# archinetai/audio-diffusion-pytorch

Measured on NVIDIA B200. Metric: audio-seconds/sec (2ch, 2^18 len) VSampler 50-step, higher is better.
Workload: dtype bf16

## Files before the change

audio_diffusion_pytorch_b200/csrc/conv_gemm.cu:

```cuda
#include <type_traits>

#include "common.cuh"
#include "ptx.cuh"

namespace adp {

int g_debug[8] = {2, 1, 0, 0, 0, 0, 0, 0};

constexpr int kBM = 128;
constexpr int kMaxStages = 8;
constexpr int kMaxGroups = 8;

struct Gemm2Params {
  __nv_bfloat16* out;
  const __nv_bfloat16* residual;
  const float* bias;
  const float* gate;
  double* stats;
  int B, T, tiles_per_batch, c_in, ldo;
  int n_pad, n_valid;
  int ntaps, tap_off0, up_factor;
  int groups, group_size, group_shift;
  int out_fp32, ld_gate;
  int n_tiles_n, total_tiles, tiles_per_cta;
// ... 558 lines not shown
  if (BN != 128 || SW != 128 || XF || g_debug[0] != 3) return false;
  const int taps = a.up_factor > 1 ? 2 : a.ntaps;
  const long m_tiles = (long)a.B * ((a.T + kBM - 1) / kBM);
  return m_tiles >= 2 && (a.c_in / 64) * taps >= 8;
}

template <int BN, int SW, bool XF>
static int launch_gemm2(const adp_conv_gemm_args& a, cudaStream_t stream) {
  if constexpr (BN == 128 && SW == 128 && !XF) {
    if (use_pairs<BN, SW, XF>(a)) {
      const long m_pairs = ((long)a.B * ((a.T + kBM - 1) / kBM) + 1) / 2;
      const long total = m_pairs * (a.phases * a.n_pad / BN);
      if (g_debug[7] == 0 && 2 * total <= 2L * num_sms()) return launch_gemm2_ew<BN, SW, XF, 8, 2>(a, stream, 1);
      return launch_gemm2_ew<BN, SW, XF, 4, 2>(a, stream, 1);
    }
  }
  return launch_gemm2_ew<BN, SW, XF, 4>(a, stream, 0);
}

template <int BN, int SW, bool XF, int EW, int CG>
static int launch_gemm2_ew(const adp_conv_gemm_args& a, cudaStream_t stream, int occ_in) {
  constexpr int BK = SW / 2;
  constexpr int WN = BN / CG;
  const int tiles_per_batch = (a.T + kBM - 1) / kBM;
  const bool up = a.up_factor > 1;
  const int max_taps = up ? 2 : a.ntaps;
  const int span = up ? 1 : a.ntaps - 1;
  const int a_rows = kBM + span;
  const int k_chunks = a.c_in / BK;

  Gemm2Params p;
  p.a_sub_bytes = (a_rows * SW + 1023) / 1024 * 1024;
  p.w_sub_bytes = (WN * SW + 1023) / 1024 * 1024;
  p.max_taps = max_taps;
  const int chunk_bytes = p.a_sub_bytes + max_taps * p.w_sub_bytes;

  const int w_iters = k_chunks * max_taps;
  int occ = 1;
  if (BN <= 64 && w_iters <= 8) occ = 3;
  else if (BN <= 128 && w_iters <= 12) occ = 2;
  if (XF && occ > (BN <= 64 ? 2 : 1)) occ = BN <= 64 ? 2 : 1;
  if (g_debug[3] > 0) occ = g_debug[3];
  if (occ_in > 0) occ = occ_in;
  const int tmem_occ = 512 / (2 * (BN < 32 ? 32 : BN));
  if (occ > tmem_occ) occ = tmem_occ;
  auto budget_of = [](int o) {
    return (o == 1 ? (EW == 8 ? 204 : 196) : (o == 2 ? (XF ? 92 : 96) : 60)) * 1024;
  };
  while (occ > 1 && budget_of(occ) < 2 * chunk_bytes) --occ;
  if constexpr (EW == 4 && !XF && BN >= 64 && CG == 1) {
    const long total = (long)a.B * tiles_per_batch * (a.phases * a.n_pad / BN);
    if (g_debug[7] == 0 && ((occ == 1 && total <= 2L * num_sms()) || total <= (long)num_sms()))
      return launch_gemm2_ew<BN, SW, XF, 8>(a, stream, 1);
  }
  const int budget = budget_of(occ);
  int kc = 1;
  while (kc * 2 <= 4 && k_chunks % (kc * 2) == 0 && kc * max_taps * (BK / 16) < 8 &&
         2 * (kc * 2) * chunk_bytes <= budget)
    kc *= 2;
  if (g_debug[5] > 0 && k_chunks % g_debug[5] == 0) kc = g_debug[5];
  p.kc = kc;
  p.k_stages = k_chunks / kc;
  p.stage_bytes = kc * chunk_bytes;
  int n_stages = budget / p.stage_bytes;
  if (n_stages > kMaxStages) n_stages = kMaxStages;
  if (n_stages < 2)
    return set_error("adp_conv_gemm: stage of %d bytes does not fit (BN=%d)", p.stage_bytes, BN);
  p.n_stages = n_stages;
  const size_t smem = static_cast<size_t>(n_stages) * p.stage_bytes + 1024;

  CUtensorMap tmA, tmW;
  {
    const uint64_t dims[3] = {(uint64_t)a.c_in, (uint64_t)a.T, (uint64_t)a.B};
    const uint64_t strides[2] = {(uint64_t)a.lda * 2, (uint64_t)a.T * a.lda * 2};
    const uint32_t box[3] = {(uint32_t)BK, (uint32_t)a_rows, 1};
    if (int e = make_tmap_bf16(&tmA, a.a, 3, dims, strides, box, SW)) return e;
  }
  {
    const uint64_t dims[2] = {(uint64_t)a.k_total, (uint64_t)a.phases * a.n_pad};
    const uint64_t strides[1] = {(uint64_t)a.k_total * 2};
    const uint32_t box[2] = {(uint32_t)BK, (uint32_t)WN};
    if (int e = make_tmap_bf16(&tmW, a.w, 2, dims, strides, box, SW)) return e;
  }

  static SmemAttrCache smem_cache;
  ADP_CUDA(ensure_dyn_smem(conv_gemm2_kernel<BN, SW, XF, EW, CG>, smem, smem_cache));

  p.out = static_cast<__nv_bfloat16*>(a.out);
  p.residual = static_cast<const __nv_bfloat16*>(a.residual);
  p.bias = a.bias;
  p.gate = a.gate;
  p.stats = a.stats;
  p.B = a.B;
  p.T = a.T;
  p.tiles_per_batch = tiles_per_batch;
  p.c_in = a.c_in;
  p.ldo = a.ldo;
  p.n_pad = a.n_pad;
  p.n_valid = a.n_valid;
  p.ntaps = a.ntaps;
  p.tap_off0 = a.tap_off[0];
  p.up_factor = a.up_factor;
  p.groups = a.stats ? a.groups : 0;
  p.group_size = a.stats ? a.n_valid / a.groups : 1;
  p.group_shift = -1;
  for (int sft = 0; sft < 16; ++sft)
    if ((1 << sft) == p.group_size) p.group_shift = sft;
  p.out_fp32 = a.out_fp32;
  p.ld_gate = a.ld_gate > 0 ? a.ld_gate : a.n_valid;
  p.n_tiles_n = a.phases * a.n_pad / BN;
  p.total_tiles = (a.B * tiles_per_batch + CG - 1) / CG * p.n_tiles_n;
  p.a_rows = a_rows;
  p.dbg = g_debug[4];
  p.early_w = g_debug[2];
  p.gn_stats = a.gn_stats;
  p.gn_gamma = a.gn_gamma;
  p.gn_beta = a.gn_beta;
  p.gn_eps = a.gn_eps;
  p.gn_groups = a.gn_groups > 0 ? a.gn_groups : 1;

  const int slots = occ * num_sms() / CG;
  int grid = p.total_tiles < slots ? p.total_tiles : slots;
  p.tiles_per_cta = (p.total_tiles + grid - 1) / grid;
  grid = (p.total_tiles + p.tiles_per_cta - 1) / p.tiles_per_cta;
  ADP_CUDA(launch_k_cluster(conv_gemm2_kernel<BN, SW, XF, EW, CG>, dim3(grid * CG),
                            dim3(64 + 32 * EW + (XF ? 256 : 0)), smem, stream, CG, tmA, tmW, p));
  ADP_LAUNCH_CHECK();
  return 0;
}

template <int SW>
static int dispatch_bn2(const adp_conv_gemm_args& a, int bn, cudaStream_t s) {
  if (a.gn_stats) {
    switch (bn) {
      case 16: return launch_gemm2<16, SW, true>(a, s);
      case 32: return launch_gemm2<32, SW, true>(a, s);
      case 64: return launch_gemm2<64, SW, true>(a, s);
      case 128: return launch_gemm2<128, SW, true>(a, s);
      case 256: return launch_gemm2<256, SW, true>(a, s);
    }
  }
  switch (bn) {
    case 16: return launch_gemm2<16, SW, false>(a, s);
    case 32: return launch_gemm2<32, SW, false>(a, s);
    case 64: return launch_gemm2<64, SW, false>(a, s);
    case 128: return launch_gemm2<128, SW, false>(a, s);
    case 256: return launch_gemm2<256, SW, false>(a, s);
  }
  return set_error("adp_conv_gemm: unsupported N tile %d", bn);
}

}

namespace adp { extern int g_mid_threads; }

extern "C" int adp_debug_set(int key, int value) {
  if (key == 8) {
    if (value != 128 && value != 256) return adp::set_error("adp_debug_set: key 8 takes 128 or 256");
    adp::g_mid_threads = value;
    return 0;
  }
  if (key < 0 || key >= 8) return adp::set_error("adp_debug_set: bad key %d", key);
  adp::g_debug[key] = value;
  if (key == 6) adp::g_pdl = value;
  return 0;
}

extern "C" int adp_conv_gemm(const adp_conv_gemm_args* args, adp_stream_t stream) {
  using namespace adp;
  ADP_CHECK(args != nullptr, "adp_conv_gemm: null args");
  const adp_conv_gemm_args& a = *args;
  ADP_CHECK(a.a && a.w && a.out, "adp_conv_gemm: null a/w/out");
  ADP_CHECK(a.B > 0 && a.T > 0, "adp_conv_gemm: bad B=%d T=%d", a.B, a.T);
  ADP_CHECK(a.c_in >= 16 && a.c_in % 16 == 0, "adp_conv_gemm: c_in=%d must be a multiple of 16",
            a.c_in);
  ADP_CHECK(a.lda % 8 == 0 && a.ldo % 8 == 0 && a.k_total % 8 == 0 && a.lda >= a.c_in,
            "adp_conv_gemm: pitches lda=%d ldo=%d k_total=%d must be multiples of 8", a.lda, a.ldo,
            a.k_total);
  ADP_CHECK(a.n_valid > 0 && a.n_valid % 8 == 0 && a.n_valid <= a.n_pad && a.n_pad % 16 == 0,
            "adp_conv_gemm: n_valid=%d n_pad=%d", a.n_valid, a.n_pad);
  ADP_CHECK(a.phases >= 1, "adp_conv_gemm: phases=%d", a.phases);
  ADP_CHECK(a.ld_gate % 4 == 0, "adp_conv_gemm: ld_gate=%d must be a multiple of 4", a.ld_gate);
  if (a.up_factor > 1) {
    ADP_CHECK(a.phases == a.up_factor, "adp_conv_gemm: phases (%d) != up_factor (%d)", a.phases,
              a.up_factor);
    ADP_CHECK(a.k_total >= 2 * a.c_in, "adp_conv_gemm: upsample weights need 2 tap slots");
  } else {
    ADP_CHECK(a.ntaps >= 1 && a.ntaps <= 3 && a.phases == 1, "adp_conv_gemm: ntaps=%d phases=%d",
              a.ntaps, a.phases);
    ADP_CHECK(a.k_total >= a.ntaps * a.c_in, "adp_conv_gemm: k_total too small");
    for (int i = 1; i < a.ntaps; ++i)
      ADP_CHECK(a.tap_off[i] == a.tap_off[i - 1] + 1,
                "adp_conv_gemm: tap offsets must be consecutive and ascending");
  }
  if (a.out_fp32) {
    ADP_CHECK(!a.residual && !a.stats, "adp_conv_gemm: out_fp32 excludes residual/stats");
  }
  if (a.gn_stats) {
    ADP_CHECK(a.c_in <= 1024, "adp_conv_gemm: fused GroupNorm supports c_in <= 1024");
    ADP_CHECK(a.gn_gamma && a.gn_beta && a.gn_groups > 0 && a.c_in % a.gn_groups == 0 && a.lda == a.c_in,
              "adp_conv_gemm: fused GroupNorm needs gamma/beta, groups | c_in and a dense input");
  }
  if (a.stats) {
    ADP_CHECK(a.groups > 0 && a.groups <= kMaxGroups && a.n_valid % a.groups == 0,
              "adp_conv_gemm: groups=%d n_valid=%d (fused statistics handle <= %d groups)",
              a.groups, a.n_valid, kMaxGroups);
  }
  int bn = a.block_n;
  if (bn == 0) {
    const long m_tiles = (long)a.B * ((a.T + kBM - 1) / kBM);
    bn = 16;
    for (int cand = 128; cand >= 16; cand >>= 1) {
      if (a.n_pad % cand) continue;
      const long tiles = m_tiles * (a.phases * a.n_pad / cand);
      if (tiles >= 96 || cand <= 64) { bn = cand; break; }
    }
  }
  ADP_CHECK(a.n_pad % bn == 0, "adp_conv_gemm: N tile %d does not divide n_pad %d", bn, a.n_pad);
  cudaStream_t s = as_stream(stream);
  if (a.c_in % 64 == 0) return dispatch_bn2<128>(a, bn, s);
  if (a.c_in % 32 == 0) return dispatch_bn2<64>(a, bn, s);
  return dispatch_bn2<32>(a, bn, s);
}
```

audio_diffusion_pytorch_b200/csrc/mid_conv.cu:

```cuda
#include "common.cuh"
#include "ptx.cuh"

namespace adp {

__device__ __forceinline__ void ldsm_x4(uint32_t addr, uint32_t (&r)[4]) {
  asm volatile("ldmatrix.sync.aligned.m8n8.x4.shared.b16 {%0,%1,%2,%3}, [%4];"
               : "=r"(r[0]), "=r"(r[1]), "=r"(r[2]), "=r"(r[3]) : "r"(addr));
}
__device__ __forceinline__ void mma_bf16_16816(float (&d)[4], const uint32_t (&a)[4], uint32_t b0,
                                               uint32_t b1) {
  asm volatile(
      "mma.sync.aligned.m16n8k16.row.col.f32.bf16.bf16.f32 {%0,%1,%2,%3}, {%4,%5,%6,%7}, {%8,%9}, "
      "{%0,%1,%2,%3};"
      : "+f"(d[0]), "+f"(d[1]), "+f"(d[2]), "+f"(d[3])
      : "r"(a[0]), "r"(a[1]), "r"(a[2]), "r"(a[3]), "r"(b0), "r"(b1));
}

template <int C, int NTH>
struct MidCfg {
  static constexpr int TB = (C == 32 ? 256 : 128) * NTH / 256;
  static constexpr int TPR = NTH / TB;
  static constexpr int RPW = TB / (NTH / 32);
  static constexpr int RS = C * 2 + 16;
  static constexpr int WS = 3 * C * 2 + 16;
  static constexpr int MB = RPW / 16;
  static constexpr int NT = C / 8;
  static constexpr int OS = C + 4;
  static constexpr int LPR = C / 8;
  static constexpr int ER = TB * LPR / NTH;
  static constexpr int X_BYTES = (TB + 2) * RS;
  static constexpr int O_BYTES = TB * OS * 4;
  static constexpr int W_BYTES = C * WS;
  static constexpr int SMEM = X_BYTES + O_BYTES + W_BYTES;
};

template <int C, int NTH>
__global__ void __launch_bounds__(NTH, 512 / NTH) mid_conv_kernel(const adp_narrow_conv_args a) {
  using Cfg = MidCfg<C, NTH>;
  constexpr int TB = Cfg::TB, TPR = Cfg::TPR, RS = Cfg::RS, WS = Cfg::WS, MB = Cfg::MB, NT = Cfg::NT;
  constexpr int OS = Cfg::OS, LPR = Cfg::LPR, ER = Cfg::ER, RPW = Cfg::RPW;
  pdl_launch_dependents();
  pdl_wait();
  extern __shared__ __align__(128) uint8_t smem[];
  uint8_t* s_x = smem;
  float* s_o = reinterpret_cast<float*>(smem + Cfg::X_BYTES);
  uint8_t* s_w = smem + Cfg::X_BYTES + Cfg::O_BYTES;
  __shared__ __align__(16) float s_ga[C], s_de[C];
  __shared__ __align__(16) float s_sc[C], s_sh[C];
  __shared__ float s_bias[C];
  __shared__ float s_stats[2 * 64];
  const int b = blockIdx.y;
  const int tid = threadIdx.x;
  const int warp = tid >> 5, lane = tid & 31;
  const int g = lane >> 2, q = lane & 3;
  const bool has_res = a.residual != nullptr, has_film = a.scale_shift != nullptr;

  if (tid < 128) s_stats[tid] = 0.f;
  if (a.w_packed) {
    constexpr int VPRW = 3 * C * 2 / 16;
    const uint4* wp = static_cast<const uint4*>(a.w_packed);
    for (int i = tid; i < C * VPRW; i += NTH) {
      const int co = i / VPRW, v = i - co * VPRW;
      *reinterpret_cast<uint4*>(s_w + co * WS + v * 16) = __ldg(wp + i);
    }
  } else {
    for (int pidx = tid; pidx < C * C; pidx += NTH) {
      const int co = pidx / C, ci = pidx % C;
      const float* src = a.w + static_cast<size_t>(pidx) * 3;
#pragma unroll
      for (int tap = 0; tap < 3; ++tap)
        *reinterpret_cast<__nv_bfloat16*>(s_w + co * WS + (tap * C + ci) * 2) = __float2bfloat16(src[tap]);
    }
  }
  if (tid < C) {
    const int c = tid;
    const int gsz = C / a.groups, gi = c / gsz;
    const double inv_n = 1.0 / (static_cast<double>(gsz) * a.T);
    const double sm = a.stats_in[(static_cast<size_t>(b) * a.groups + gi) * 2];
    const double sq = a.stats_in[(static_cast<size_t>(b) * a.groups + gi) * 2 + 1];
    const double mean = sm * inv_n;
    const float var = fmaxf(static_cast<float>(sq * inv_n - mean * mean), 0.f);
    const float ga = a.gamma[c] * rsqrtf(var + a.gn_eps);
    s_ga[c] = ga;
    s_de[c] = a.beta[c] - static_cast<float>(mean) * ga;
    s_bias[c] = a.bias ? a.bias[c] : 0.f;
    const float* ss = has_film ? a.scale_shift + static_cast<size_t>(b) * a.ss_stride : nullptr;
    s_sc[c] = has_film ? 1.f + ss[c] : 1.f;
    s_sh[c] = has_film ? ss[C + c] : 0.f;
  }
  __syncthreads();

  const __nv_bfloat16* xb = static_cast<const __nv_bfloat16*>(a.x) + static_cast<size_t>(b) * a.T * C;
  const __nv_bfloat16* rb =
      has_res ? static_cast<const __nv_bfloat16*>(a.residual) + static_cast<size_t>(b) * a.T * C : nullptr;
  __nv_bfloat16* yb = static_cast<__nv_bfloat16*>(a.y) + static_cast<size_t>(b) * a.T * C;
  const int n_tiles = (a.T + TB - 1) / TB;

  const int srow = tid / TPR, spart = tid % TPR;
  const int el = tid % LPR, erow0 = tid / LPR;
  float fsc[8], fsh[8];
#pragma unroll
  for (int j = 0; j < 8; ++j) { fsc[j] = s_sc[el * 8 + j]; fsh[j] = s_sh[el * 8 + j]; }

  auto load_tile = [&](int tile, uint4 (&xr)[4], uint4 (&hr)[4]) {
    const int t0 = tile * TB;
    const int t = t0 + srow;
#pragma unroll
    for (int i = 0; i < 4; ++i) {
      xr[i] = make_uint4(0, 0, 0, 0);
      hr[i] = make_uint4(0, 0, 0, 0);
    }
    if (t < a.T) {
      const uint4* p = reinterpret_cast<const uint4*>(xb + static_cast<size_t>(t) * C + spart * 32);
#pragma unroll
      for (int i = 0; i < 4; ++i) xr[i] = __ldg(p + i);
    }
    if (tid < 2 * TPR) {
      const int th = tid < TPR ? t0 - 1 : t0 + TB;
      if (th >= 0 && th < a.T) {
        const uint4* p = reinterpret_cast<const uint4*>(xb + static_cast<size_t>(th) * C + (tid % TPR) * 32);
#pragma unroll
        for (int i = 0; i < 4; ++i) hr[i] = __ldg(p + i);
      }
    }
  };
  auto activate = [&](const uint4& u, int c8, bool valid) {
    if (!valid) return make_uint4(0, 0, 0, 0);
    const float4 a0 = *reinterpret_cast<const float4*>(&s_ga[spart * 32 + c8]);
    const float4 a1 = *reinterpret_cast<const float4*>(&s_ga[spart * 32 + c8 + 4]);
    const float4 d0 = *reinterpret_cast<const float4*>(&s_de[spart * 32 + c8]);
    const float4 d1 = *reinterpret_cast<const float4*>(&s_de[spart * 32 + c8 + 4]);
    const float2 f0 = unpack_bf16(u.x), f1 = unpack_bf16(u.y), f2 = unpack_bf16(u.z), f3 = unpack_bf16(u.w);
    uint4 o;
    o.x = pack_bf16(silu_fast(f0.x * a0.x + d0.x), silu_fast(f0.y * a0.y + d0.y));
    o.y = pack_bf16(silu_fast(f1.x * a0.z + d0.z), silu_fast(f1.y * a0.w + d0.w));
    o.z = pack_bf16(silu_fast(f2.x * a1.x + d1.x), silu_fast(f2.y * a1.y + d1.y));
    o.w = pack_bf16(silu_fast(f3.x * a1.z + d1.z), silu_fast(f3.y * a1.w + d1.w));
    return o;
  };

  float st_s[2] = {0.f, 0.f}, st_q[2] = {0.f, 0.f};

  int tile = blockIdx.x;
  uint4 xr[4], hr[4];
  if (tile < n_tiles) load_tile(tile, xr, hr);
  const uint32_t w_base = smem_u32(s_w);
  const uint32_t x_base = smem_u32(s_x);
  for (; tile < n_tiles; tile += gridDim.x) {
    const int t0 = tile * TB;
    {
      const bool valid = t0 + srow < a.T;
#pragma unroll
      for (int i = 0; i < 4; ++i)
        *reinterpret_cast<uint4*>(s_x + (srow + 1) * RS + spart * 64 + i * 16) = activate(xr[i], i * 8, valid);
      if (tid < 2 * TPR) {
        const int th = tid < TPR ? t0 - 1 : t0 + TB;
        const bool hv = th >= 0 && th < a.T;
        uint8_t* dst = s_x + (tid < TPR ? 0 : TB + 1) * RS + (tid % TPR) * 64;
#pragma unroll
        for (int i = 0; i < 4; ++i) *reinterpret_cast<uint4*>(dst + i * 16) = activate(hr[i], i * 8, hv);
      }
    }
    if (tile + gridDim.x < n_tiles) load_tile(tile + gridDim.x, xr, hr);
    uint4 res[ER];
    if (has_res) {
#pragma unroll
      for (int i = 0; i < ER; ++i) {
        const int t = t0 + erow0 + i * (NTH / LPR);
        res[i] = make_uint4(0, 0, 0, 0);
        if (t < a.T) res[i] = __ldg(reinterpret_cast<const uint4*>(rb + static_cast<size_t>(t) * C + el * 8));
      }
    }
    __syncthreads();

    float acc[MB][NT][4];
#pragma unroll
    for (int mb = 0; mb < MB; ++mb)
#pragma unroll
      for (int j = 0; j < NT; ++j) {
        acc[mb][j][0] = s_bias[8 * j + 2 * q]; acc[mb][j][1] = s_bias[8 * j + 2 * q + 1];
        acc[mb][j][2] = acc[mb][j][0]; acc[mb][j][3] = acc[mb][j][1];
      }
#pragma unroll
    for (int tap = 0; tap < 3; ++tap) {
#pragma unroll
      for (int c16 = 0; c16 < C / 16; ++c16) {
        uint32_t af[MB][4];
#pragma unroll
        for (int mb = 0; mb < MB; ++mb) {
          const int r0 = warp * RPW + mb * 16;
          ldsm_x4(x_base + static_cast<uint32_t>(r0 + (lane & 7) + ((lane >> 3) & 1) * 8 + tap) * RS +
                      (c16 * 16 + ((lane >> 4) & 1) * 8) * 2, af[mb]);
        }
#pragma unroll
        for (int np = 0; np < NT / 2; ++np) {
          uint32_t bf[4];
          ldsm_x4(w_base + static_cast<uint32_t>(np * 16 + (lane & 7) + ((lane >> 4) & 1) * 8) * WS +
                      (tap * C + c16 * 16 + ((lane >> 3) & 1) * 8) * 2, bf);
#pragma unroll
          for (int mb = 0; mb < MB; ++mb) {
            mma_bf16_16816(acc[mb][2 * np], af[mb], bf[0], bf[1]);
            mma_bf16_16816(acc[mb][2 * np + 1], af[mb], bf[2], bf[3]);
          }
        }
      }
    }
#pragma unroll
    for (int mb = 0; mb < MB; ++mb) {
      const int r = warp * RPW + mb * 16 + g;
#pragma unroll
      for (int j = 0; j < NT; ++j) {
        *reinterpret_cast<float2*>(s_o + r * OS + 8 * j + 2 * q) = make_float2(acc[mb][j][0], acc[mb][j][1]);
        *reinterpret_cast<float2*>(s_o + (r + 8) * OS + 8 * j + 2 * q) = make_float2(acc[mb][j][2], acc[mb][j][3]);
      }
    }
    __syncthreads();

#pragma unroll
    for (int i = 0; i < ER; ++i) {
      const int rl = erow0 + i * (NTH / LPR);
      const int t = t0 + rl;
      const float4 o0 = *reinterpret_cast<const float4*>(s_o + rl * OS + el * 8);
      const float4 o1 = *reinterpret_cast<const float4*>(s_o + rl * OS + el * 8 + 4);
      float y[8] = {o0.x, o0.y, o0.z, o0.w, o1.x, o1.y, o1.z, o1.w};
      if (has_res) {
        const float2 r0 = unpack_bf16(res[i].x), r1 = unpack_bf16(res[i].y);
        const float2 r2 = unpack_bf16(res[i].z), r3 = unpack_bf16(res[i].w);
        y[0] += r0.x; y[1] += r0.y; y[2] += r1.x; y[3] += r1.y;
        y[4] += r2.x; y[5] += r2.y; y[6] += r3.x; y[7] += r3.y;
      }
      if (has_film) {
        float m = ((y[0] + y[1]) + (y[2] + y[3])) + ((y[4] + y[5]) + (y[6] + y[7]));
#pragma unroll
        for (int o = LPR >> 1; o > 0; o >>= 1) m += __shfl_xor_sync(0xffffffffu, m, o);
        m *= (1.f / C);
        float v = 0.f;
#pragma unroll
        for (int j = 0; j < 8; ++j) { y[j] -= m; v += y[j] * y[j]; }
#pragma unroll
        for (int o = LPR >> 1; o > 0; o >>= 1) v += __shfl_xor_sync(0xffffffffu, v, o);
        const float rstd = rsqrtf(v * (1.f / C) + a.ln_eps);
#pragma unroll
        for (int j = 0; j < 8; ++j) y[j] = y[j] * rstd * fsc[j] + fsh[j];
      }
      uint4 ov;
      ov.x = pack_bf16(y[0], y[1]); ov.y = pack_bf16(y[2], y[3]);
      ov.z = pack_bf16(y[4], y[5]); ov.w = pack_bf16(y[6], y[7]);
      if (t < a.T) {
        *reinterpret_cast<uint4*>(yb + static_cast<size_t>(t) * C + el * 8) = ov;
        const float2 q0 = unpack_bf16(ov.x), q1 = unpack_bf16(ov.y);
        const float2 q2 = unpack_bf16(ov.z), q3 = unpack_bf16(ov.w);
        st_s[0] += (q0.x + q0.y) + (q1.x + q1.y);
        st_q[0] += (q0.x * q0.x + q0.y * q0.y) + (q1.x * q1.x + q1.y * q1.y);
        st_s[1] += (q2.x + q2.y) + (q3.x + q3.y);
        st_q[1] += (q2.x * q2.x + q2.y * q2.y) + (q3.x * q3.x + q3.y * q3.y);
      }
    }
  }
  if (a.stats_out) {
    const int gsz = C / a.groups;
#pragma unroll
    for (int hf = 0; hf < 2; ++hf) {
#pragma unroll
      for (int o = LPR; o < 32; o <<= 1) {
        st_s[hf] += __shfl_xor_sync(0xffffffffu, st_s[hf], o);
        st_q[hf] += __shfl_xor_sync(0xffffffffu, st_q[hf], o);
      }
      if (lane < LPR) {
        const int gi = (el * 8 + hf * 4) / gsz;
        atomicAdd(&s_stats[2 * gi], st_s[hf]);
        atomicAdd(&s_stats[2 * gi + 1], st_q[hf]);
      }
    }
    __syncthreads();
    if (tid < 2 * a.groups && s_stats[tid] != 0.f)
      atomicAdd(a.stats_out + static_cast<size_t>(b) * 2 * a.groups + tid, static_cast<double>(s_stats[tid]));
  }
}

int g_mid_threads = 256;

template <int C, int NTH>
static int launch_mid(const adp_narrow_conv_args& a, cudaStream_t stream) {
  using Cfg = MidCfg<C, NTH>;
  static SmemAttrCache smem_cache;
  ADP_CUDA(ensure_dyn_smem(mid_conv_kernel<C, NTH>, (size_t)Cfg::SMEM, smem_cache));
  int dev = 0, sms = 148, occ = 1;
  cudaGetDevice(&dev);
  cudaDeviceGetAttribute(&sms, cudaDevAttrMultiProcessorCount, dev);
  if (cudaOccupancyMaxActiveBlocksPerMultiprocessor(&occ, mid_conv_kernel<C, NTH>, NTH, Cfg::SMEM) != cudaSuccess ||
      occ < 1)
    occ = 1;
  const int n_tiles = (a.T + Cfg::TB - 1) / Cfg::TB;
  int gx = (occ * sms) / a.B;
  if (gx < 1) gx = 1;
  if (gx > n_tiles) gx = n_tiles;
  ADP_CUDA(launch_k(mid_conv_kernel<C, NTH>, dim3(gx, a.B), dim3(NTH), (size_t)Cfg::SMEM, stream, a));
  return 0;
}

int mid_conv(const adp_narrow_conv_args& a, cudaStream_t stream) {
  const bool small = g_mid_threads == 128;
  if (a.C == 32) return small ? launch_mid<32, 128>(a, stream) : launch_mid<32, 256>(a, stream);
  if (a.C == 64) return small ? launch_mid<64, 128>(a, stream) : launch_mid<64, 256>(a, stream);
  return set_error("adp_narrow_conv: C=%d is not built (8, 32, 64)", a.C);
}

}
```

Measured before the change: 243.4.

## Rewrite narrow mid conv as warp-specialized TMA/tcgen05 persistent pipeline

Replaces the mma.sync-based mid-channel conv kernel with a persistent, warp-specialized kernel. A TMA producer warp loads input and residual tiles, four warps apply GroupNorm+SiLU in place in swizzled shared memory, and a single MMA warp issues tcgen05 UMMA into multi-buffered TMEM accumulators. One or two epilogue groups add bias and residual, apply FiLM layernorm and stats, and store output with TMA. The goal is to overlap loads, normalization, MMA and epilogue across tiles. The cost is more complex mbarrier synchronization and higher shared-memory use, and the old 128/256-thread debug knob is removed.

```diff
diff --git a/audio_diffusion_pytorch_b200/csrc/conv_gemm.cu b/audio_diffusion_pytorch_b200/csrc/conv_gemm.cu
--- a/audio_diffusion_pytorch_b200/csrc/conv_gemm.cu
+++ b/audio_diffusion_pytorch_b200/csrc/conv_gemm.cu
@@ -734,14 +734,7 @@
 
 }
 
-namespace adp { extern int g_mid_threads; }
-
 extern "C" int adp_debug_set(int key, int value) {
-  if (key == 8) {
-    if (value != 128 && value != 256) return adp::set_error("adp_debug_set: key 8 takes 128 or 256");
-    adp::g_mid_threads = value;
-    return 0;
-  }
   if (key < 0 || key >= 8) return adp::set_error("adp_debug_set: bad key %d", key);
   adp::g_debug[key] = value;
   if (key == 6) adp::g_pdl = value;
diff --git a/audio_diffusion_pytorch_b200/csrc/mid_conv.cu b/audio_diffusion_pytorch_b200/csrc/mid_conv.cu
--- a/audio_diffusion_pytorch_b200/csrc/mid_conv.cu
+++ b/audio_diffusion_pytorch_b200/csrc/mid_conv.cu
@@ -3,306 +3,441 @@
 
 namespace adp {
 
-__device__ __forceinline__ void ldsm_x4(uint32_t addr, uint32_t (&r)[4]) {
-  asm volatile("ldmatrix.sync.aligned.m8n8.x4.shared.b16 {%0,%1,%2,%3}, [%4];"
-               : "=r"(r[0]), "=r"(r[1]), "=r"(r[2]), "=r"(r[3]) : "r"(addr));
-}
-__device__ __forceinline__ void mma_bf16_16816(float (&d)[4], const uint32_t (&a)[4], uint32_t b0,
-                                               uint32_t b1) {
+__device__ __forceinline__ void tma_store_3d(const CUtensorMap* m, const void* smem_src, int c0, int c1, int c2) {
   asm volatile(
-      "mma.sync.aligned.m16n8k16.row.col.f32.bf16.bf16.f32 {%0,%1,%2,%3}, {%4,%5,%6,%7}, {%8,%9}, "
-      "{%0,%1,%2,%3};"
-      : "+f"(d[0]), "+f"(d[1]), "+f"(d[2]), "+f"(d[3])
-      : "r"(a[0]), "r"(a[1]), "r"(a[2]), "r"(a[3]), "r"(b0), "r"(b1));
-}
-
-template <int C, int NTH>
-struct MidCfg {
-  static constexpr int TB = (C == 32 ? 256 : 128) * NTH / 256;
-  static constexpr int TPR = NTH / TB;
-  static constexpr int RPW = TB / (NTH / 32);
-  static constexpr int RS = C * 2 + 16;
-  static constexpr int WS = 3 * C * 2 + 16;
-  static constexpr int MB = RPW / 16;
-  static constexpr int NT = C / 8;
-  static constexpr int OS = C + 4;
-  static constexpr int LPR = C / 8;
-  static constexpr int ER = TB * LPR / NTH;
-  static constexpr int X_BYTES = (TB + 2) * RS;
-  static constexpr int O_BYTES = TB * OS * 4;
-  static constexpr int W_BYTES = C * WS;
-  static constexpr int SMEM = X_BYTES + O_BYTES + W_BYTES;
+      "cp.async.bulk.tensor.3d.global.shared::cta.bulk_group [%0, {%2, %3, %4}], [%1];" ::"l"(
+          reinterpret_cast<uint64_t>(m)),
+      "r"(smem_u32(smem_src)), "r"(c0), "r"(c1), "r"(c2)
+      : "memory");
+}
+__device__ __forceinline__ void bulk_commit_group() {
+  asm volatile("cp.async.bulk.commit_group;" ::: "memory");
+}
+template <int N>
+__device__ __forceinline__ void bulk_wait_group_read() {
+  asm volatile("cp.async.bulk.wait_group.read %0;" ::"n"(N) : "memory");
+}
+__device__ __forceinline__ void bulk_wait_group_all() {
+  asm volatile("cp.async.bulk.wait_group 0;" ::: "memory");
+}
+
+template <int C>
+struct ThinCfg {
+  static constexpr int SW = 2 * C;
+  static constexpr int CPR = SW / 16;
+  static constexpr int TM = 128;
+  static constexpr int A_ROWS = TM + 2;
+  static constexpr int A_STAGE = (A_ROWS * SW + 1023) / 1024 * 1024;
+  static constexpr int R_STAGE = TM * SW;
+  static constexpr int O_WARP = 32 * SW;
+  static constexpr int W_TAP = C * SW;
+  static constexpr int NA = C == 32 ? 6 : 4;
+  static constexpr int NR = C == 32 ? 4 : 3;
+  static constexpr int EG = C == 32 ? 2 : 1;
+  static constexpr int THREADS = 192 + 128 * EG;
+  static constexpr int SMEM_A = 0;
+  static constexpr int SMEM_R = SMEM_A + NA * A_STAGE;
+  static constexpr int SMEM_O = SMEM_R + NR * R_STAGE;
+  static constexpr int SMEM_W = SMEM_O + 2 * 4 * EG * O_WARP;
+  static constexpr int SMEM = SMEM_W + 3 * W_TAP + 1024;
 };
-
-template <int C, int NTH>
-__global__ void __launch_bounds__(NTH, 512 / NTH) mid_conv_kernel(const adp_narrow_conv_args a) {
-  using Cfg = MidCfg<C, NTH>;
-  constexpr int TB = Cfg::TB, TPR = Cfg::TPR, RS = Cfg::RS, WS = Cfg::WS, MB = Cfg::MB, NT = Cfg::NT;
-  constexpr int OS = Cfg::OS, LPR = Cfg::LPR, ER = Cfg::ER, RPW = Cfg::RPW;
+constexpr int kAcc = 4;
+constexpr int kThinMaxGroups = 16;
+
+struct ThinParams {
+  adp_narrow_conv_args a;
+  int tiles_per_batch, total_tiles, tiles_per_cta;
+  int early_w;
+};
+
+template <int SW>
+__device__ __forceinline__ uint32_t swz_off(int row, int lc) {
+  const uint32_t off = static_cast<uint32_t>(row) * SW;
+  return off + ((lc ^ ((off >> 7) & (SW / 16 - 1))) << 4);
+}
+
+template <int C, bool RES, bool FILM, int SL>
+__global__ void __launch_bounds__(ThinCfg<C>::THREADS, 1)
+thin_conv_kernel(const __grid_constant__ CUtensorMap tmX, const __grid_constant__ CUtensorMap tmR,
+                 const __grid_constant__ CUtensorMap tmY, const ThinParams p) {
+  using Cfg = ThinCfg<C>;
+  constexpr int SW = Cfg::SW, CPR = Cfg::CPR, NA = Cfg::NA, NR = Cfg::NR, EG = Cfg::EG;
+  extern __shared__ uint8_t smem_raw[];
+  __shared__ uint64_t a_full[NA], a_ready[NA], a_empty[NA];
+  __shared__ uint64_t r_full[NR], r_empty[NR];
+  __shared__ uint64_t acc_full[kAcc], acc_empty[kAcc];
+  __shared__ uint32_t tmem_slot;
+  __shared__ __align__(16) float s_ga[C], s_de[C];
+  __shared__ __align__(16) float s_sc[EG][C], s_sh[EG][C];
+  __shared__ __align__(16) float s_bias[C];
+  __shared__ float s_stats[EG][2 * kThinMaxGroups];
+  const adp_narrow_conv_args& a = p.a;
+
   pdl_launch_dependents();
-  pdl_wait();
-  extern __shared__ __align__(128) uint8_t smem[];
-  uint8_t* s_x = smem;
-  float* s_o = reinterpret_cast<float*>(smem + Cfg::X_BYTES);
-  uint8_t* s_w = smem + Cfg::X_BYTES + Cfg::O_BYTES;
-  __shared__ __align__(16) float s_ga[C], s_de[C];
-  __shared__ __align__(16) float s_sc[C], s_sh[C];
-  __shared__ float s_bias[C];
-  __shared__ float s_stats[2 * 64];
-  const int b = blockIdx.y;
-  const int tid = threadIdx.x;
-  const int warp = tid >> 5, lane = tid & 31;
-  const int g = lane >> 2, q = lane & 3;
-  const bool has_res = a.residual != nullptr, has_film = a.scale_shift != nullptr;
-
-  if (tid < 128) s_stats[tid] = 0.f;
-  if (a.w_packed) {
-    constexpr int VPRW = 3 * C * 2 / 16;
-    const uint4* wp = static_cast<const uint4*>(a.w_packed);
-    for (int i = tid; i < C * VPRW; i += NTH) {
-      const int co = i / VPRW, v = i - co * VPRW;
-      *reinterpret_cast<uint4*>(s_w + co * WS + v * 16) = __ldg(wp + i);
+  const int warp = warp_id_uniform();
+  const int lane = threadIdx.x & 31;
+  const uint32_t raw = smem_u32(smem_raw);
+  uint8_t* base = smem_raw + ((1024u - (raw & 1023u)) & 1023u);
+  uint8_t* s_a = base + Cfg::SMEM_A;
+  uint8_t* s_r = base + Cfg::SMEM_R;
+  uint8_t* s_o = base + Cfg::SMEM_O;
+  uint8_t* s_w = base + Cfg::SMEM_W;
+
+  const int tile_begin = blockIdx.x * p.tiles_per_cta;
+  const int tile_end = min(tile_begin + p.tiles_per_cta, p.total_tiles);
+
+  if (warp == 0) {
+    tmem_alloc(&tmem_slot, kAcc * C);
+    tmem_relinquish();
+  } else if (warp == 1 && lane == 0) {
+    for (int s = 0; s < NA; ++s) { mbar_init(&a_full[s], 1); mbar_init(&a_ready[s], 128); mbar_init(&a_empty[s], 1); }
+    static_assert(EG == 1 || NR % EG == 0, "a residual stage must always serve the same epilogue group");
+    for (int s = 0; s < NR; ++s) { mbar_init(&r_full[s], 1); mbar_init(&r_empty[s], 4); }
+    for (int s = 0; s < kAcc; ++s) { mbar_init(&acc_full[s], 1); mbar_init(&acc_empty[s], 4); }
+    fence_mbar_init();
+    tma_prefetch_desc(&tmX);
+    if (RES) tma_prefetch_desc(&tmR);
+    tma_prefetch_desc(&tmY);
+  }
+  if (!p.early_w) pdl_wait();
+  {
+    constexpr int VPR = 3 * CPR;
+    for (int i = threadIdx.x; i < C * VPR; i += Cfg::THREADS) {
+      const int co = i / VPR, v = i - co * VPR;
+      const int tap = v / CPR, lc = v - tap * CPR;
+      uint4 u;
+      if (a.w_packed) {
+        u = __ldg(static_cast<const uint4*>(a.w_packed) + i);
+      } else {
+        const float* src = a.w + (static_cast<size_t>(co) * C + lc * 8) * 3 + tap;
+        u.x = pack_bf16(src[0], src[3]);
+        u.y = pack_bf16(src[6], src[9]);
+        u.z = pack_bf16(src[12], src[15]);
+        u.w = pack_bf16(src[18], src[21]);
+      }
+      *reinterpret_cast<uint4*>(s_w + tap * Cfg::W_TAP + swz_off<SW>(co, lc)) = u;
+    }
+  }
+  for (int i = threadIdx.x; i < C; i += Cfg::THREADS) s_bias[i] = a.bias ? a.bias[i] : 0.f;
+  for (int i = threadIdx.x; i < EG * 2 * kThinMaxGroups; i += Cfg::THREADS) (&s_stats[0][0])[i] = 0.f;
+  fence_proxy_async_smem();
+  tc_fence_before();
+  __syncthreads();
+  tc_fence_after();
+  const uint32_t tmem_base = __shfl_sync(0xffffffffu, tmem_slot, 0);
+
+  if (warp == 0) {
+    pdl_wait();
+    int s = 0, rs = 0;
+    uint32_t ph = 0, rph = 0;
+    for (int tile = tile_begin; tile < tile_end; ++tile) {
+      const int b = tile / p.tiles_per_batch;
+      const int t0 = (tile - b * p.tiles_per_batch) * Cfg::TM;
+      mbar_wait(&a_empty[s], ph ^ 1);
+      if (elect_one()) {
+        mbar_arrive_expect_tx(&a_full[s], Cfg::A_ROWS * SW);
+        tma_load_3d(s_a + s * Cfg::A_STAGE, &tmX, &a_full[s], 0, t0 - 1, b);
+      }
+      __syncwarp();
+      if (++s == NA) { s = 0; ph ^= 1; }
+      if constexpr (RES) {
+        mbar_wait(&r_empty[rs], rph ^ 1);
+        if (elect_one()) {
+          mbar_arrive_expect_tx(&r_full[rs], Cfg::R_STAGE);
+          tma_load_3d(s_r + rs * Cfg::R_STAGE, &tmR, &r_full[rs], 0, t0, b);
+        }
+        __syncwarp();
+        if (++rs == NR) { rs = 0; rph ^= 1; }
+      }
+    }
+  } else if (warp == 1) {
+    constexpr uint32_t idesc = umma_idesc_bf16(Cfg::TM, C, 0, 0);
+    const uint64_t adesc0 = umma_desc_kmajor<SW>(smem_u32(s_a));
+    const uint64_t wdesc0 = umma_desc_kmajor<SW>(smem_u32(s_w));
+    int s = 0;
+    uint32_t ph = 0, j = 0;
+    for (int tile = tile_begin; tile < tile_end; ++tile, ++j) {
+      const uint32_t buf = j % kAcc;
+      mbar_wait(&acc_empty[buf], ((j / kAcc) & 1) ^ 1);
+      mbar_wait(&a_ready[s], ph);
+      tc_fence_after();
+      if (elect_one()) {
+        const uint32_t d_tmem = tmem_base + buf * C;
+        const uint64_t adesc = adesc0 + static_cast<uint64_t>((s * Cfg::A_STAGE) >> 4);
+#pragma unroll
+        for (int tap = 0; tap < 3; ++tap)
+#pragma unroll
+          for (int kk = 0; kk < C / 16; ++kk)
+            umma_bf16(d_tmem, adesc + ((tap * SW + kk * 32) >> 4),
+                      wdesc0 + ((tap * Cfg::W_TAP + kk * 32) >> 4), idesc, (tap | kk) != 0);
+        umma_commit(&a_empty[s]);
+        umma_commit(&acc_full[buf]);
+      }
+      __syncwarp();
+      if (++s == NA) { s = 0; ph ^= 1; }
+    }
+  } else if (warp < 6) {
+    pdl_wait();
+    const int tt = threadIdx.x - 64;
+    const int lc = tt % CPR;
+    const int r0 = tt / CPR;
+    constexpr int RSTEP = 128 / CPR;
+    const int gsz = C / a.groups;
+    const double inv_n = 1.0 / (static_cast<double>(gsz) * a.T);
+    float ga[8], de[8];
+    int s = 0, cur_b = -1;
+    uint32_t ph = 0;
+    for (int tile = tile_begin; tile < tile_end; ++tile) {
+      const int b = tile / p.tiles_per_batch;
+      const int t0 = (tile - b * p.tiles_per_batch) * Cfg::TM;
+      if (b != cur_b) {
+        named_bar_sync(1, 128);
+        if (tt < C) {
+          const int gi = tt / gsz;
+          const double mean = a.stats_in[(static_cast<size_t>(b) * a.groups + gi) * 2] * inv_n;
+          const double sq = a.stats_in[(static_cast<size_t>(b) * a.groups + gi) * 2 + 1];
+          const float var = fmaxf(static_cast<float>(sq * inv_n - mean * mean), 0.f);
+          const float g = a.gamma[tt] * rsqrtf(var + a.gn_eps);
+          s_ga[tt] = g;
+          s_de[tt] = a.beta[tt] - static_cast<float>(mean) * g;
+        }
+        named_bar_sync(1, 128);
+#pragma unroll
+        for (int i = 0; i < 8; ++i) { ga[i] = s_ga[lc * 8 + i]; de[i] = s_de[lc * 8 + i]; }
+        cur_b = b;
+      }
+      mbar_wait(&a_full[s], ph);
+      uint8_t* st = s_a + s * Cfg::A_STAGE;
+#pragma unroll 2
+      for (int rr = r0; rr < Cfg::A_ROWS; rr += RSTEP) {
+        const int t = t0 - 1 + rr;
+        if (t < 0 || t >= a.T) continue;
+        uint4* ptr = reinterpret_cast<uint4*>(st + swz_off<SW>(rr, lc));
+        const uint4 u = *ptr;
+        const float2 f0 = unpack_bf16(u.x), f1 = unpack_bf16(u.y);
+        const float2 f2 = unpack_bf16(u.z), f3 = unpack_bf16(u.w);
+        uint4 o;
+        o.x = pack_bf16(silu_fast(f0.x * ga[0] + de[0]), silu_fast(f0.y * ga[1] + de[1]));
+        o.y = pack_bf16(silu_fast(f1.x * ga[2] + de[2]), silu_fast(f1.y * ga[3] + de[3]));
+        o.z = pack_bf16(silu_fast(f2.x * ga[4] + de[4]), silu_fast(f2.y * ga[5] + de[5]));
+        o.w = pack_bf16(silu_fast(f3.x * ga[6] + de[6]), silu_fast(f3.y * ga[7] + de[7]));
+        *ptr = o;
+      }
+      fence_proxy_async_smem();
+      mbar_arrive(&a_ready[s]);
+      if (++s == NA) { s = 0; ph ^= 1; }
     }
   } else {
-    for (int pidx = tid; pidx < C * C; pidx += NTH) {
-      const int co = pidx / C, ci = pidx % C;
-      const float* src = a.w + static_cast<size_t>(pidx) * 3;
-#pragma unroll
-      for (int tap = 0; tap < 3; ++tap)
-        *reinterpret_cast<__nv_bfloat16*>(s_w + co * WS + (tap * C + ci) * 2) = __float2bfloat16(src[tap]);
-    }
-  }
-  if (tid < C) {
-    const int c = tid;
-    const int gsz = C / a.groups, gi = c / gsz;
-    const double inv_n = 1.0 / (static_cast<double>(gsz) * a.T);
-    const double sm = a.stats_in[(static_cast<size_t>(b) * a.groups + gi) * 2];
-    const double sq = a.stats_in[(static_cast<size_t>(b) * a.groups + gi) * 2 + 1];
-    const double mean = sm * inv_n;
-    const float var = fmaxf(static_cast<float>(sq * inv_n - mean * mean), 0.f);
-    const float ga = a.gamma[c] * rsqrtf(var + a.gn_eps);
-    s_ga[c] = ga;
-    s_de[c] = a.beta[c] - static_cast<float>(mean) * ga;
-    s_bias[c] = a.bias ? a.bias[c] : 0.f;
-    const float* ss = has_film ? a.scale_shift + static_cast<size_t>(b) * a.ss_stride : nullptr;
-    s_sc[c] = has_film ? 1.f + ss[c] : 1.f;
-    s_sh[c] = has_film ? ss[C + c] : 0.f;
-  }
+    pdl_wait();
+    const int q = warp & 3;
+    const int row = q * 32 + lane;
+    const int eg = (warp - 6) >> 2;
+    const int et = (threadIdx.x - 192) & 127;
+    float* bins = s_stats[eg];
+    const float* f_sc = s_sc[eg];
+    const float* f_sh = s_sh[eg];
+    const uint32_t lane_addr = static_cast<uint32_t>(q * 32) << 16;
+    const bool do_stats = a.stats_out != nullptr;
+    const int gsz = C / a.groups;
+    constexpr int NSLOT = C / SL;
+    float st_s[NSLOT], st_q[NSLOT];
+#pragma unroll
+    for (int i = 0; i < NSLOT; ++i) { st_s[i] = 0.f; st_q[i] = 0.f; }
+    uint8_t* o_warp = s_o + (warp - 6) * 2 * Cfg::O_WARP;
+
+    auto fold_stats = [&]() {
+#pragma unroll
+      for (int i = 0; i < NSLOT; ++i) {
+        const float ws = warp_sum(st_s[i]), wq = warp_sum(st_q[i]);
+        if (lane == 0) {
+          const int gi = (i * SL) / gsz;
+          atomicAdd(&bins[2 * gi], ws);
+          atomicAdd(&bins[2 * gi + 1], wq);
+        }
+        st_s[i] = 0.f; st_q[i] = 0.f;
+      }
+    };
+    auto publish_stats = [&](int b_done) {
+      if (et < 2 * a.groups) {
+        const float v = bins[et];
+        if (v != 0.f) atomicAdd(a.stats_out + static_cast<size_t>(b_done) * 2 * a.groups + et, static_cast<double>(v));
+        bins[et] = 0.f;
+      }
+    };
+
+    int rs = eg, cur_b = -1;
+    uint32_t rph = 0, j = eg;
+    for (int tile = tile_begin + eg; tile < tile_end; tile += EG, j += EG) {
+      const int b = tile / p.tiles_per_batch;
+      const int t0 = (tile - b * p.tiles_per_batch) * Cfg::TM;
+      if (b != cur_b) {
+        if (do_stats && cur_b >= 0) fold_stats();
+        named_bar_sync(2 + eg, 128);
+        if (do_stats && cur_b >= 0) publish_stats(cur_b);
+        if (FILM && et < C) {
+          const float* ss = a.scale_shift + static_cast<size_t>(b) * a.ss_stride;
+          s_sc[eg][et] = 1.f + ss[et];
+          s_sh[eg][et] = ss[C + et];
+        }
+        named_bar_sync(2 + eg, 128);
+        cur_b = b;
+      }
+      const uint32_t buf = j % kAcc;
+      mbar_wait(&acc_full[buf], (j / kAcc) & 1);
+      tc_fence_after();
+      float v[C];
+      {
+        uint32_t r[C];
+        const uint32_t taddr = tmem_base + buf * C + lane_addr;
+#pragma unroll
+        for (int h = 0; h < C / 32; ++h)
+          tmem_ld32(taddr + h * 32, *reinterpret_cast<uint32_t(*)[32]>(r + h * 32));
+        tmem_ld_wait();
+#pragma unroll
+        for (int c = 0; c < C; ++c) v[c] = __uint_as_float(r[c]);
+      }
+      tc_fence_before();
+      __syncwarp();
+      if (lane == 0) mbar_arrive(&acc_empty[buf]);
+#pragma unroll
+      for (int c = 0; c < C; c += 4) {
+        const float4 bb = *reinterpret_cast<const float4*>(&s_bias[c]);
+        v[c] += bb.x; v[c + 1] += bb.y; v[c + 2] += bb.z; v[c + 3] += bb.w;
+      }
+      if constexpr (RES) {
+        mbar_wait(&r_full[rs], rph);
+        const uint8_t* rrow = s_r + rs * Cfg::R_STAGE;
+#pragma unroll
+        for (int lc = 0; lc < CPR; ++lc) {
+          const uint4 u = *reinterpret_cast<const uint4*>(rrow + swz_off<SW>(row, lc));
+          const float2 r0 = unpack_bf16(u.x), r1 = unpack_bf16(u.y);
+          const float2 r2 = unpack_bf16(u.z), r3 = unpack_bf16(u.w);
+          float* w8 = v + lc * 8;
+          w8[0] += r0.x; w8[1] += r0.y; w8[2] += r1.x; w8[3] += r1.y;
+          w8[4] += r2.x; w8[5] += r2.y; w8[6] += r3.x; w8[7] += r3.y;
+        }
+        __syncwarp();
+        if (lane == 0) mbar_arrive(&r_empty[rs]);
+        if ((rs += EG) >= NR) { rs -= NR; rph ^= 1; }
+      }
+      if constexpr (FILM) {
+        float m4[4] = {0.f, 0.f, 0.f, 0.f};
+#pragma unroll
+        for (int c = 0; c < C; ++c) m4[c & 3] += v[c];
+        const float m = ((m4[0] + m4[1]) + (m4[2] + m4[3])) * (1.f / C);
+        float q4[4] = {0.f, 0.f, 0.f, 0.f};
+#pragma unroll
+        for (int c = 0; c < C; ++c) { v[c] -= m; q4[c & 3] += v[c] * v[c]; }
+        const float var = (q4[0] + q4[1]) + (q4[2] + q4[3]);
+        const float rstd = rsqrtf(var * (1.f / C) + a.ln_eps);
+#pragma unroll
+        for (int c = 0; c < C; c += 4) {
+          const float4 sc = *reinterpret_cast<const float4*>(&f_sc[c]);
+          const float4 sh = *reinterpret_cast<const float4*>(&f_sh[c]);
+          v[c] = v[c] * rstd * sc.x + sh.x; v[c + 1] = v[c + 1] * rstd * sc.y + sh.y;
+          v[c + 2] = v[c + 2] * rstd * sc.z + sh.z; v[c + 3] = v[c + 3] * rstd * sc.w + sh.w;
+        }
+      }
+      uint8_t* ob = o_warp + ((j / EG) & 1) * Cfg::O_WARP;
+      if (lane == 0) bulk_wait_group_read<1>();
+      __syncwarp();
+      const bool row_ok = t0 + row < a.T;
+#pragma unroll
+      for (int lc = 0; lc < CPR; ++lc) {
+        const float* w8 = v + lc * 8;
+        uint4 o;
+        o.x = pack_bf16(w8[0], w8[1]); o.y = pack_bf16(w8[2], w8[3]);
+        o.z = pack_bf16(w8[4], w8[5]); o.w = pack_bf16(w8[6], w8[7]);
+        *reinterpret_cast<uint4*>(ob + swz_off<SW>(lane, lc)) = o;
+        if (do_stats && row_ok) {
+          const float2 q0 = unpack_bf16(o.x), q1 = unpack_bf16(o.y);
+          const float2 q2 = unpack_bf16(o.z), q3 = unpack_bf16(o.w);
+          const float s0 = (q0.x + q0.y) + (q1.x + q1.y), s1 = (q2.x + q2.y) + (q3.x + q3.y);
+          const float e0 = (q0.x * q0.x + q0.y * q0.y) + (q1.x * q1.x + q1.y * q1.y);
+          const float e1 = (q2.x * q2.x + q2.y * q2.y) + (q3.x * q3.x + q3.y * q3.y);
+          if constexpr (SL == 8) {
+            st_s[lc] += s0 + s1;
+            st_q[lc] += e0 + e1;
+          } else {
+            st_s[2 * lc] += s0; st_q[2 * lc] += e0;
+            st_s[2 * lc + 1] += s1; st_q[2 * lc + 1] += e1;
+          }
+        }
+      }
+      fence_proxy_async_smem();
+      __syncwarp();
+      if (lane == 0) {
+        if (t0 + q * 32 < a.T) tma_store_3d(&tmY, ob, 0, t0 + q * 32, b);
+        bulk_commit_group();
+      }
+      __syncwarp();
+    }
+    if (do_stats && cur_b >= 0) {
+      fold_stats();
+      named_bar_sync(2 + eg, 128);
+      publish_stats(cur_b);
+    }
+    if (lane == 0) bulk_wait_group_all();
+  }
+
+  tc_fence_before();
   __syncthreads();
-
-  const __nv_bfloat16* xb = static_cast<const __nv_bfloat16*>(a.x) + static_cast<size_t>(b) * a.T * C;
-  const __nv_bfloat16* rb =
-      has_res ? static_cast<const __nv_bfloat16*>(a.residual) + static_cast<size_t>(b) * a.T * C : nullptr;
-  __nv_bfloat16* yb = static_cast<__nv_bfloat16*>(a.y) + static_cast<size_t>(b) * a.T * C;
-  const int n_tiles = (a.T + TB - 1) / TB;
-
-  const int srow = tid / TPR, spart = tid % TPR;
-  const int el = tid % LPR, erow0 = tid / LPR;
-  float fsc[8], fsh[8];
-#pragma unroll
-  for (int j = 0; j < 8; ++j) { fsc[j] = s_sc[el * 8 + j]; fsh[j] = s_sh[el * 8 + j]; }
-
-  auto load_tile = [&](int tile, uint4 (&xr)[4], uint4 (&hr)[4]) {
-    const int t0 = tile * TB;
-    const int t = t0 + srow;
-#pragma unroll
-    for (int i = 0; i < 4; ++i) {
-      xr[i] = make_uint4(0, 0, 0, 0);
-      hr[i] = make_uint4(0, 0, 0, 0);
-    }
-    if (t < a.T) {
-      const uint4* p = reinterpret_cast<const uint4*>(xb + static_cast<size_t>(t) * C + spart * 32);
-#pragma unroll
-      for (int i = 0; i < 4; ++i) xr[i] = __ldg(p + i);
-    }
-    if (tid < 2 * TPR) {
-      const int th = tid < TPR ? t0 - 1 : t0 + TB;
-      if (th >= 0 && th < a.T) {
-        const uint4* p = reinterpret_cast<const uint4*>(xb + static_cast<size_t>(th) * C + (tid % TPR) * 32);
-#pragma unroll
-        for (int i = 0; i < 4; ++i) hr[i] = __ldg(p + i);
-      }
-    }
-  };
-  auto activate = [&](const uint4& u, int c8, bool valid) {
-    if (!valid) return make_uint4(0, 0, 0, 0);
-    const float4 a0 = *reinterpret_cast<const float4*>(&s_ga[spart * 32 + c8]);
-    const float4 a1 = *reinterpret_cast<const float4*>(&s_ga[spart * 32 + c8 + 4]);
-    const float4 d0 = *reinterpret_cast<const float4*>(&s_de[spart * 32 + c8]);
-    const float4 d1 = *reinterpret_cast<const float4*>(&s_de[spart * 32 + c8 + 4]);
-    const float2 f0 = unpack_bf16(u.x), f1 = unpack_bf16(u.y), f2 = unpack_bf16(u.z), f3 = unpack_bf16(u.w);
-    uint4 o;
-    o.x = pack_bf16(silu_fast(f0.x * a0.x + d0.x), silu_fast(f0.y * a0.y + d0.y));
-    o.y = pack_bf16(silu_fast(f1.x * a0.z + d0.z), silu_fast(f1.y * a0.w + d0.w));
-    o.z = pack_bf16(silu_fast(f2.x * a1.x + d1.x), silu_fast(f2.y * a1.y + d1.y));
-    o.w = pack_bf16(silu_fast(f3.x * a1.z + d1.z), silu_fast(f3.y * a1.w + d1.w));
-    return o;
-  };
-
-  float st_s[2] = {0.f, 0.f}, st_q[2] = {0.f, 0.f};
-
-  int tile = blockIdx.x;
-  uint4 xr[4], hr[4];
-  if (tile < n_tiles) load_tile(tile, xr, hr);
-  const uint32_t w_base = smem_u32(s_w);
-  const uint32_t x_base = smem_u32(s_x);
-  for (; tile < n_tiles; tile += gridDim.x) {
-    const int t0 = tile * TB;
-    {
-      const bool valid = t0 + srow < a.T;
-#pragma unroll
-      for (int i = 0; i < 4; ++i)
-        *reinterpret_cast<uint4*>(s_x + (srow + 1) * RS + spart * 64 + i * 16) = activate(xr[i], i * 8, valid);
-      if (tid < 2 * TPR) {
-        const int th = tid < TPR ? t0 - 1 : t0 + TB;
-        const bool hv = th >= 0 && th < a.T;
-        uint8_t* dst = s_x + (tid < TPR ? 0 : TB + 1) * RS + (tid % TPR) * 64;
-#pragma unroll
-        for (int i = 0; i < 4; ++i) *reinterpret_cast<uint4*>(dst + i * 16) = activate(hr[i], i * 8, hv);
-      }
-    }
-    if (tile + gridDim.x < n_tiles) load_tile(tile + gridDim.x, xr, hr);
-    uint4 res[ER];
-    if (has_res) {
-#pragma unroll
-      for (int i = 0; i < ER; ++i) {
-        const int t = t0 + erow0 + i * (NTH / LPR);
-        res[i] = make_uint4(0, 0, 0, 0);
-        if (t < a.T) res[i] = __ldg(reinterpret_cast<const uint4*>(rb + static_cast<size_t>(t) * C + el * 8));
-      }
-    }
-    __syncthreads();
-
-    float acc[MB][NT][4];
-#pragma unroll
-    for (int mb = 0; mb < MB; ++mb)
-#pragma unroll
-      for (int j = 0; j < NT; ++j) {
-        acc[mb][j][0] = s_bias[8 * j + 2 * q]; acc[mb][j][1] = s_bias[8 * j + 2 * q + 1];
-        acc[mb][j][2] = acc[mb][j][0]; acc[mb][j][3] = acc[mb][j][1];
-      }
-#pragma unroll
-    for (int tap = 0; tap < 3; ++tap) {
-#pragma unroll
-      for (int c16 = 0; c16 < C / 16; ++c16) {
-        uint32_t af[MB][4];
-#pragma unroll
-        for (int mb = 0; mb < MB; ++mb) {
-          const int r0 = warp * RPW + mb * 16;
-          ldsm_x4(x_base + static_cast<uint32_t>(r0 + (lane & 7) + ((lane >> 3) & 1) * 8 + tap) * RS +
-                      (c16 * 16 + ((lane >> 4) & 1) * 8) * 2, af[mb]);
-        }
-#pragma unroll
-        for (int np = 0; np < NT / 2; ++np) {
-          uint32_t bf[4];
-          ldsm_x4(w_base + static_cast<uint32_t>(np * 16 + (lane & 7) + ((lane >> 4) & 1) * 8) * WS +
-                      (tap * C + c16 * 16 + ((lane >> 3) & 1) * 8) * 2, bf);
-#pragma unroll
-          for (int mb = 0; mb < MB; ++mb) {
-            mma_bf16_16816(acc[mb][2 * np], af[mb], bf[0], bf[1]);
-            mma_bf16_16816(acc[mb][2 * np + 1], af[mb], bf[2], bf[3]);
-          }
-        }
-      }
-    }
-#pragma unroll
-    for (int mb = 0; mb < MB; ++mb) {
-      const int r = warp * RPW + mb * 16 + g;
-#pragma unroll
-      for (int j = 0; j < NT; ++j) {
-        *reinterpret_cast<float2*>(s_o + r * OS + 8 * j + 2 * q) = make_float2(acc[mb][j][0], acc[mb][j][1]);
-        *reinterpret_cast<float2*>(s_o + (r + 8) * OS + 8 * j + 2 * q) = make_float2(acc[mb][j][2], acc[mb][j][3]);
-      }
-    }
-    __syncthreads();
-
-#pragma unroll
-    for (int i = 0; i < ER; ++i) {
-      const int rl = erow0 + i * (NTH / LPR);
-      const int t = t0 + rl;
-      const float4 o0 = *reinterpret_cast<const float4*>(s_o + rl * OS + el * 8);
-      const float4 o1 = *reinterpret_cast<const float4*>(s_o + rl * OS + el * 8 + 4);
-      float y[8] = {o0.x, o0.y, o0.z, o0.w, o1.x, o1.y, o1.z, o1.w};
-      if (has_res) {
-        const float2 r0 = unpack_bf16(res[i].x), r1 = unpack_bf16(res[i].y);
-        const float2 r2 = unpack_bf16(res[i].z), r3 = unpack_bf16(res[i].w);
-        y[0] += r0.x; y[1] += r0.y; y[2] += r1.x; y[3] += r1.y;
-        y[4] += r2.x; y[5] += r2.y; y[6] += r3.x; y[7] += r3.y;
-      }
-      if (has_film) {
-        float m = ((y[0] + y[1]) + (y[2] + y[3])) + ((y[4] + y[5]) + (y[6] + y[7]));
-#pragma unroll
-        for (int o = LPR >> 1; o > 0; o >>= 1) m += __shfl_xor_sync(0xffffffffu, m, o);
-        m *= (1.f / C);
-        float v = 0.f;
-#pragma unroll
-        for (int j = 0; j < 8; ++j) { y[j] -= m; v += y[j] * y[j]; }
-#pragma unroll
-        for (int o = LPR >> 1; o > 0; o >>= 1) v += __shfl_xor_sync(0xffffffffu, v, o);
-        const float rstd = rsqrtf(v * (1.f / C) + a.ln_eps);
-#pragma unroll
-        for (int j = 0; j < 8; ++j) y[j] = y[j] * rstd * fsc[j] + fsh[j];
-      }
-      uint4 ov;
-      ov.x = pack_bf16(y[0], y[1]); ov.y = pack_bf16(y[2], y[3]);
-      ov.z = pack_bf16(y[4], y[5]); ov.w = pack_bf16(y[6], y[7]);
-      if (t < a.T) {
-        *reinterpret_cast<uint4*>(yb + static_cast<size_t>(t) * C + el * 8) = ov;
-        const float2 q0 = unpack_bf16(ov.x), q1 = unpack_bf16(ov.y);
-        const float2 q2 = unpack_bf16(ov.z), q3 = unpack_bf16(ov.w);
-        st_s[0] += (q0.x + q0.y) + (q1.x + q1.y);
-        st_q[0] += (q0.x * q0.x + q0.y * q0.y) + (q1.x * q1.x + q1.y * q1.y);
-        st_s[1] += (q2.x + q2.y) + (q3.x + q3.y);
-        st_q[1] += (q2.x * q2.x + q2.y * q2.y) + (q3.x * q3.x + q3.y * q3.y);
-      }
-    }
-  }
-  if (a.stats_out) {
-    const int gsz = C / a.groups;
-#pragma unroll
-    for (int hf = 0; hf < 2; ++hf) {
-#pragma unroll
-      for (int o = LPR; o < 32; o <<= 1) {
-        st_s[hf] += __shfl_xor_sync(0xffffffffu, st_s[hf], o);
-        st_q[hf] += __shfl_xor_sync(0xffffffffu, st_q[hf], o);
-      }
-      if (lane < LPR) {
-        const int gi = (el * 8 + hf * 4) / gsz;
-        atomicAdd(&s_stats[2 * gi], st_s[hf]);
-        atomicAdd(&s_stats[2 * gi + 1], st_q[hf]);
-      }
-    }
-    __syncthreads();
-    if (tid < 2 * a.groups && s_stats[tid] != 0.f)
-      atomicAdd(a.stats_out + static_cast<size_t>(b) * 2 * a.groups + tid, static_cast<double>(s_stats[tid]));
-  }
-}
-
-int g_mid_threads = 256;
-
-template <int C, int NTH>
-static int launch_mid(const adp_narrow_conv_args& a, cudaStream_t stream) {
-  using Cfg = MidCfg<C, NTH>;
+  if (warp == 0) {
+    __syncwarp();
+    tmem_dealloc(tmem_base, kAcc * C);
+  }
+}
+
+extern int g_debug[8];
+
+template <int C, bool RES, bool FILM, int SL>
+static int launch_thin(const adp_narrow_conv_args& a, cudaStream_t stream) {
+  using Cfg = ThinCfg<C>;
+  const uint64_t dims[3] = {(uint64_t)C, (uint64_t)a.T, (uint64_t)a.B};
+  const uint64_t strides[2] = {(uint64_t)C * 2, (uint64_t)a.T * C * 2};
+  CUtensorMap tmX, tmR, tmY;
+  {
+    const uint32_t box[3] = {(uint32_t)C, (uint32_t)Cfg::A_ROWS, 1};
+    if (int e = make_tmap_bf16(&tmX, a.x, 3, dims, strides, box, Cfg::SW)) return e;
+  }
+  {
+    const uint32_t box[3] = {(uint32_t)C, (uint32_t)Cfg::TM, 1};
+    if (int e = make_tmap_bf16(&tmR, RES ? a.residual : a.x, 3, dims, strides, box, Cfg::SW)) return e;
+  }
+  {
+    const uint32_t box[3] = {(uint32_t)C, 32, 1};
+    if (int e = make_tmap_bf16(&tmY, a.y, 3, dims, strides, box, Cfg::SW)) return e;
+  }
   static SmemAttrCache smem_cache;
-  ADP_CUDA(ensure_dyn_smem(mid_conv_kernel<C, NTH>, (size_t)Cfg::SMEM, smem_cache));
-  int dev = 0, sms = 148, occ = 1;
-  cudaGetDevice(&dev);
-  cudaDeviceGetAttribute(&sms, cudaDevAttrMultiProcessorCount, dev);
-  if (cudaOccupancyMaxActiveBlocksPerMultiprocessor(&occ, mid_conv_kernel<C, NTH>, NTH, Cfg::SMEM) != cudaSuccess ||
-      occ < 1)
-    occ = 1;
-  const int n_tiles = (a.T + Cfg::TB - 1) / Cfg::TB;
-  int gx = (occ * sms) / a.B;
-  if (gx < 1) gx = 1;
-  if (gx > n_tiles) gx = n_tiles;
-  ADP_CUDA(launch_k(mid_conv_kernel<C, NTH>, dim3(gx, a.B), dim3(NTH), (size_t)Cfg::SMEM, stream, a));
+  ADP_CUDA(ensure_dyn_smem(thin_conv_kernel<C, RES, FILM, SL>, (size_t)Cfg::SMEM, smem_cache));
+  int dev = 0, sms = 0;
+  ADP_CUDA(cudaGetDevice(&dev));
+  ADP_CUDA(cudaDeviceGetAttribute(&sms, cudaDevAttrMultiProcessorCount, dev));
+  if (sms <= 0) sms = 148;
+  ThinParams p;
+  p.a = a;
+  p.early_w = g_debug[2];
+  p.tiles_per_batch = (a.T + Cfg::TM - 1) / Cfg::TM;
+  p.total_tiles = a.B * p.tiles_per_batch;
+  int grid = p.total_tiles < sms ? p.total_tiles : sms;
+  p.tiles_per_cta = (p.total_tiles + grid - 1) / grid;
+  grid = (p.total_tiles + p.tiles_per_cta - 1) / p.tiles_per_cta;
+  ADP_CUDA(launch_k(thin_conv_kernel<C, RES, FILM, SL>, dim3(grid), dim3(Cfg::THREADS), (size_t)Cfg::SMEM, stream,
+                    tmX, tmR, tmY, p));
   return 0;
 }
 
+template <int C, int SL>
+static int dispatch_thin(const adp_narrow_conv_args& a, cudaStream_t stream) {
+  const bool res = a.residual != nullptr, film = a.scale_shift != nullptr;
+  if (res) return film ? launch_thin<C, true, true, SL>(a, stream) : launch_thin<C, true, false, SL>(a, stream);
+  return film ? launch_thin<C, false, true, SL>(a, stream) : launch_thin<C, false, false, SL>(a, stream);
+}
+
 int mid_conv(const adp_narrow_conv_args& a, cudaStream_t stream) {
-  const bool small = g_mid_threads == 128;
-  if (a.C == 32) return small ? launch_mid<32, 128>(a, stream) : launch_mid<32, 256>(a, stream);
-  if (a.C == 64) return small ? launch_mid<64, 128>(a, stream) : launch_mid<64, 256>(a, stream);
+  const bool slot8 = !a.stats_out || (a.C / a.groups) % 8 == 0;
+  if (a.C == 32) return dispatch_thin<32, 4>(a, stream);
+  if (a.C == 64) return slot8 ? dispatch_thin<64, 8>(a, stream) : dispatch_thin<64, 4>(a, stream);
   return set_error("adp_narrow_conv: C=%d is not built (8, 32, 64)", a.C);
 }
 
```

Result: faster. 252.7, median of 6 (+3.8%).
